# InfiniteNightmare/HNSW-Slim

Measured on AMD Instinct MI355X. Metric: QPS @ recall@10>=0.95 (SIFT-1M d=128, k=10), higher is better.
Workload: dtype f32

## Files before the change

hnsw-slim_amd/__init__.py:

```python
import ctypes
import os
import subprocess

import numpy as np

_HERE = os.path.dirname(os.path.abspath(__file__))
LIB_PATH = os.environ.get("HS_LIB", os.path.join(_HERE, "libhnsw_slim_amd.so"))

HS_KIND_HNSW, HS_KIND_SLIM, HS_KIND_SLIMQ = 0, 1, 2
HS_METRIC_L2, HS_METRIC_IP = 0, 1
HS_MODE_SLIM_IDS, HS_MODE_PQ = 0, 1
HS_ROWS_F32, HS_ROWS_F16, HS_ROWS_U8 = 0, 1, 2
HS_OK, HS_ERR_IO, HS_ERR_CORRUPT, HS_ERR_NOMEM, HS_ERR_INVALID, HS_ERR_UNSUPPORTED, HS_ERR_DEVICE, HS_ERR_CAPACITY = range(8)

EXPORTS = [
    "hs_last_error", "hs_device_count", "hs_index_load", "hs_index_load_mem", "hs_index_free", "hs_set_ef", "hs_index_info",
    "hs_set_capacity", "hs_set_exact_order", "hs_search_batch", "hs_search_batch_dev", "hs_search_check", "hs_search_batch_raw", "hs_search_batch_filtered", "hs_labels",
    "hs_build_hnsw", "hs_build_hnsw_labeled", "hs_convert_slim", "hs_rabitq_rotate", "hs_rabitq_quantize_data", "hs_rabitq_prepare_query",
    "hs_rabitq_estimate", "hs_convert_slimq", "hs_rabitq_default_tconst", "hs_slimq_set_dataset", "hs_slimq_set_tconst", "hs_slimq_get_tconst",
    "hs_slimq_search_batch", "hs_slimq_search_batch_dev", "hs_slimq_trace", "hs_slimq_prepare_debug", "hs_brute_force", "hs_brute_force_dev",
    "hs_search_batch_async", "hs_host_alloc", "hs_host_free", "hs_comm_init", "hs_comm_free", "hs_comm_size", "hs_search_batch_sharded",
    "hs_comm_results_dev", "hs_convert_slim_gpu", "hs_index_patch", "hs_index_from_host_arrays", "hs_build_rabitq_hnsw",
    "hs_convert_slimq_graph", "hs_host_device_pointer", "hs_index_set_row_format", "hs_index_row_format", "hs_rows_representable",
]
# ... 22 lines not shown


def lib():
    global _lib
    if _lib is not None:
        return _lib
    if not os.path.exists(LIB_PATH):
        raise HsError(HS_ERR_DEVICE, f"{LIB_PATH} is missing: build it with `make -C hnsw-slim_amd` "
                      "(__graft_entry__.build()); there is no CPU fallback")
    L = ctypes.CDLL(LIB_PATH)
    vp, sz, ci, u32 = ctypes.c_void_p, ctypes.c_size_t, ctypes.c_int, ctypes.c_uint32
    L.hs_last_error.restype = ctypes.c_char_p
    L.hs_device_count.restype = ci
    L.hs_index_load.argtypes = [ctypes.c_char_p, ci, ci, sz, sz, ci, ctypes.POINTER(vp)]
    L.hs_index_load_mem.argtypes = [ctypes.c_char_p, sz, ci, ci, sz, sz, ci, ctypes.POINTER(vp)]
    L.hs_index_patch.argtypes = [vp, ctypes.c_char_p, sz, ci]
    L.hs_index_from_host_arrays.argtypes = [ci, ci, sz, sz, vp, vp, vp, vp, vp, vp, u32, ctypes.c_int32, ctypes.c_int32, ci, ctypes.POINTER(vp)]
    L.hs_index_free.argtypes = [vp]
    L.hs_index_free.restype = None
    L.hs_set_ef.argtypes = [vp, sz]
    L.hs_index_info.argtypes = [vp, ctypes.POINTER(HsInfo)]
    L.hs_index_set_row_format.argtypes = [vp, ci]
    L.hs_index_row_format.argtypes = [vp]
    L.hs_rows_representable.argtypes = [vp, sz, sz, ci, ctypes.POINTER(ctypes.c_uint64)]
    L.hs_last_kernel.argtypes = [vp]
    L.hs_last_kernel.restype = ctypes.c_char_p
    L.hs_set_capacity.argtypes = [vp, u32, u32]
    L.hs_set_exact_order.argtypes = [vp, ci]
    L.hs_search_batch.argtypes = [vp, vp, sz, sz, ci, vp, vp, vp, vp, vp]
    L.hs_search_batch_dev.argtypes = [vp, vp, sz, sz, ci, vp, vp, vp, vp, vp, vp]
    L.hs_search_check.argtypes = [vp, vp]
    L.hs_debug_heap_ops.argtypes = [vp, sz, ci, u32, vp, vp, vp]
    L.hs_debug_flat_plan.argtypes = [sz, sz, sz, vp]
    L.hs_search_batch_async.argtypes = [vp, vp, sz, sz, ci, vp, vp, vp, vp, vp, vp]
    L.hs_host_alloc.restype = vp
    L.hs_host_alloc.argtypes = [sz]
    L.hs_host_free.restype = None
    L.hs_host_free.argtypes = [vp]
    L.hs_comm_init.argtypes = [ci, vp, ctypes.POINTER(vp)]
    L.hs_comm_free.restype = None
    L.hs_comm_free.argtypes = [vp]
    L.hs_comm_size.argtypes = [vp]
    L.hs_search_batch_sharded.argtypes = [vp, vp, vp, sz, sz, ci, vp, vp, vp, vp]
    L.hs_search_batch_sharded_async.argtypes = [vp, vp, vp, sz, sz, ci, vp, vp, vp, vp, ci]
    L.hs_comm_check.argtypes = [vp, vp, ci]
    L.hs_comm_slots.argtypes = [vp]
    L.hs_comm_results_dev.argtypes = [vp, ci, vp, vp, vp, vp]
    L.hs_search_batch_raw.argtypes = [vp, vp, sz, sz, ci, vp, vp, vp, vp]
    L.hs_search_batch_filtered.argtypes = [vp, vp, sz, sz, vp, vp, vp, vp, vp]
    L.hs_labels.argtypes = [vp, vp]
    L.hs_build_hnsw.argtypes = [vp, sz, sz, ci, sz, sz, ctypes.c_char_p, sz, ci, ctypes.c_char_p]
    L.hs_convert_slim.argtypes = [ctypes.c_char_p, ci, sz, ci, ctypes.c_float, ctypes.c_float, sz, sz, sz, sz, ci, ctypes.c_char_p]
    L.hs_convert_slimq_graph.argtypes = L.hs_convert_slim.argtypes
    L.hs_host_device_pointer.restype = ctypes.c_void_p
    L.hs_host_device_pointer.argtypes = [vp]
    L.hs_build_rabitq_hnsw.argtypes = [vp, sz, sz, ci, sz, sz, sz, ci, ctypes.c_char_p]
    L.hs_convert_slim_gpu.argtypes = [ctypes.c_char_p, ci, sz, ci, ctypes.c_float, ctypes.c_float, sz, sz, sz, sz, ci, ci, ctypes.c_char_p,
                                      ctypes.POINTER(ci), ctypes.POINTER(ctypes.c_double)]
    L.hs_convert_slimq.argtypes = [ctypes.c_char_p, ci, sz, vp, sz, vp, ctypes.c_uint64, ci, ctypes.c_char_p]
    L.hs_rabitq_default_tconst.restype = ctypes.c_double
    L.hs_rabitq_default_tconst.argtypes = [sz, ctypes.c_uint64]
    L.hs_slimq_set_dataset.argtypes = [vp, vp, sz, sz]
    L.hs_slimq_set_tconst.argtypes = [vp, ctypes.c_double]
    L.hs_slimq_get_tconst.restype = ctypes.c_double
    L.hs_slimq_get_tconst.argtypes = [vp]
    L.hs_slimq_search_batch.argtypes = [vp, vp, sz, sz, vp, vp, vp, vp]
# ... 49 lines not shown
    _check(lib().hs_convert_slim_gpu(hnsw_path.encode(), metric, dim, threshold_level, top_degree_percent0, top_degree_percent,
                                     top_degree_M0, low_degree_m0, top_degree_M, low_degree_m, device, threads, out_path.encode(),
                                     ctypes.byref(used), ctypes.byref(ms)))
    return bool(used.value), ms.value


def rows_representable(rows, fmt):
    r = np.ascontiguousarray(rows, np.float32)
    r = r.reshape(r.shape[0], -1) if r.ndim != 2 else r
    bad = ctypes.c_uint64(0)
    _check(lib().hs_rows_representable(r.ctypes.data, r.shape[0], r.shape[1], int(fmt), ctypes.byref(bad)))
    return None if bad.value == r.shape[0] else int(bad.value)


def debug_flat_plan(n, ef, nq):
    out = np.zeros(5, np.uint32)
    _check(lib().hs_debug_flat_plan(n, ef, nq, out.ctypes.data))
    return dict(nb=int(out[0]), mul=int(out[1]), sh=int(out[2]), bits=int(out[3]), ok=bool(out[4]))


def debug_heap_ops(ops, wave_pop=True, lds_slots=1024):
    n = len(ops)
    arr = np.zeros((max(n, 1), 3), np.uint32)
    for i, (kind, d, idv) in enumerate(ops):
        arr[i] = (kind, np.float32(d).view(np.uint32), idv)
    heap = np.zeros((n + 2, 2), np.uint32)
    pops = np.zeros((n + 2, 2), np.uint32)
    cnt = np.zeros(2, np.uint32)
    _check(lib().hs_debug_heap_ops(arr.ctypes.data, n, 1 if wave_pop else 0, lds_slots, heap.ctypes.data, pops.ctypes.data, cnt.ctypes.data))
    f = lambda a, m: [(float(a[i, 0:1].view(np.float32)[0]), int(a[i, 1])) for i in range(m)]
    return f(heap, int(cnt[0])), f(pops, int(cnt[1]))


def brute_force(base, queries, k, metric=HS_METRIC_L2, labels=None, device=0):
    b = np.ascontiguousarray(base, np.float32)
    q = np.ascontiguousarray(queries, np.float32)
    lab = None if labels is None else np.ascontiguousarray(labels, np.uint64)
    ol = np.empty((q.shape[0], k), np.uint64)
    od = np.empty((q.shape[0], k), np.float32)
    oc = np.empty(q.shape[0], np.uint32)
    _check(lib().hs_brute_force(b.ctypes.data, b.shape[0], b.shape[1], metric, None if lab is None else lab.ctypes.data, q.ctypes.data,
                                q.shape[0], k, device, ol.ctypes.data, od.ctypes.data, oc.ctypes.data))
    return ol, od, oc


def brute_force_dev(d_base, d_queries, k, d_labels_out, d_dists_out, metric=HS_METRIC_L2, d_counts=None, stream=0):
    _check(lib().hs_brute_force_dev(d_base.data_ptr(), None, d_base.shape[0], d_base.shape[1], metric, d_queries.data_ptr(),
                                    d_queries.shape[0], k, d_labels_out.data_ptr(), d_dists_out.data_ptr(),
                                    d_counts.data_ptr() if d_counts is not None else None, stream))


def convert_slimq(slim_path, metric, dim, centroids, out_path, cluster_ids=None, flip_seed=1, threads=8):
    c = np.ascontiguousarray(centroids, np.float32).reshape(-1, dim)
    cid = None if cluster_ids is None else np.ascontiguousarray(cluster_ids, np.uint32)
    _check(lib().hs_convert_slimq(slim_path.encode(), metric, dim, c.ctypes.data, c.shape[0], None if cid is None else cid.ctypes.data,
                                  flip_seed, threads, out_path.encode()))


def rabitq_default_tconst(padded_dim, seed=1):
    return lib().hs_rabitq_default_tconst(padded_dim, seed)


def rabitq_rotate(dim, flips, x):
    x = np.ascontiguousarray(x, np.float32)
    padded = (dim + 63) // 64 * 64
    flips = np.ascontiguousarray(flips, np.uint8)
# ... 312 lines not shown
```

hnsw-slim_amd/csrc/capi.cpp:

```cpp
#include <hip/hip_runtime.h>

#include <dlfcn.h>

#include <algorithm>
#include <cmath>
#include <cstdio>
#include <cstdlib>
#include <cstring>
#include <limits>
#include <map>
#include <memory>
#include <mutex>
#include <string>
#include <vector>

#include "../../include/hnsw_slim_amd.h"
#include "engine.hpp"
#include "narrow_rows.hpp"
#define HS_HAVE_GPU_CONVERT 1
#include "convert_engine.hpp"
#include "host_graph.hpp"
#include "rabitq_est.hpp"
#include "rabitq_host.hpp"
#include "slimq_engine.hpp"
// ... 671 lines not shown
}
int hs_index_row_format(const hs_index *ix) { return ix ? ix->row_fmt : ROWS_F32; }
hs_status hs_rows_representable(const float *rows, size_t n, size_t dim, int format, uint64_t *first_bad) {
  if (!first_bad || (n && dim && !rows)) return fail(HS_ERR_INVALID, "null argument");
  if (format != ROWS_F32 && format != ROWS_F16 && format != ROWS_U8) return fail(HS_ERR_INVALID, "bad row format");
  *first_bad = dim ? first_unfit(rows, n * dim, format) / dim : n;
  return HS_OK;
}

static constexpr size_t kMaxLaunchQueries = 32768;
static constexpr size_t kOrderMinQueries = 6144;

static hs_status search_dev_group(hs_index *ix, const float *d_q, size_t nq, size_t k, int mode, uint32_t *l32,
                                  uint64_t *l64, float *dd, uint32_t *cnt, uint32_t *stats, Pair *raw, uint32_t *rawsz,
                                  hipStream_t stream, bool first_group, size_t nq_total) {
  if (!ix) return fail(HS_ERR_INVALID, "null index");
  if (k == 0) return fail(HS_ERR_INVALID, "k must be > 0");
  if (mode != HS_MODE_SLIM_IDS && mode != HS_MODE_PQ) return fail(HS_ERR_INVALID, "bad mode");
  if (ix->info.kind == HS_KIND_SLIMQ) return fail(HS_ERR_INVALID, "SlimQ index: use hs_slimq_search_batch");
  if (mode == HS_MODE_SLIM_IDS && ix->info.kind != HS_KIND_SLIM)
    return fail(HS_ERR_INVALID, "HS_MODE_SLIM_IDS needs a Slim index (searchKnn(q,k,tableint*) exists on HierarchicalNSWSlim only)");
  if (nq > 0x7FFFFFFFu) return fail(HS_ERR_INVALID, "nq too large");
  if (nq == 0) return HS_OK;
  Shape sh;
  hs_status ps = plan_shape(ix, k, sh);
  if (ps != HS_OK) return ps;
  HIP_TRY(hipSetDevice(ix->device));
  hs_index::StreamWs *w = ix->stream_ws(stream);
  HIP_TRY(w->status.ensure(nq));
  HIP_TRY(w->spill.ensure(nq * (size_t)spill_stride_for(sh.ef)));
  if (w->counters.n < 48) {
    HIP_TRY(w->counters.ensure(48));
    HIP_TRY(hipMemsetAsync(w->counters.p, 0, 48 * sizeof(uint32_t), stream));
  } else {
    HIP_TRY(hipMemsetAsync(w->counters.p + 12, 0, sizeof(uint32_t), stream));
  }
  if (first_group) w->last_nq += nq_total;
  SearchArgs a{};
  a.queries = d_q; a.nq = (uint32_t)nq; a.k = (uint32_t)k; a.ef = sh.ef;
  a.cand_cap = sh.cand_cap; a.hash_slots = sh.hash_slots; a.mode = mode;
  a.mark_ep = (ix->info.kind == HS_KIND_SLIM && mode == HS_MODE_PQ) ? 1 : 0;
  a.out_labels32 = l32; a.out_labels64 = l64; a.out_dists = dd; a.out_counts = cnt; a.stats = stats;
  a.raw_top = raw; a.raw_size = rawsz; a.raw_stride = sh.ef;
  a.status = w->status.p;
  a.spill = w->spill.p; a.spill_slots = kSpillSlots; a.spill_stride = spill_stride_for(sh.ef); a.cand2_cap = kCand2Cap;
  a.log_cap = log_cap_for(sh.ef); a.hop_cap = hop_cap_for(sh.ef);
  static const bool flat_off = getenv("HS_FLAT") && atoi(getenv("HS_FLAT")) == 0;
  a.flat = flat_off ? 0u : 1u;
  if (sh.q_bits && !ix->user_hash_slots) {
    const size_t waves_per_cu = std::max<size_t>((nq + 255) / 256, 1);
    const size_t budget = std::min<size_t>(kLdsPerCU / waves_per_cu, 64 * 1024);
    uint32_t bbits = 0;
    while ((1u << bbits) < sh.q_hash_slots / 4) bbits++;
    for (int step = 0; step < 2; step++) {
      const uint32_t bigger = sh.q_hash_slots * 2;
      const size_t lds_fast = fast_lds_bytes((uint32_t)ix->info.dim, sh.ef, sh.cand_cap_fast, bigger);
      const size_t lds_lean = lean_lds_bytes((uint32_t)ix->info.dim, sh.ef, sh.l_cand_cap, bigger);
      if (std::max(lds_fast, lds_lean) > budget || bbits + 1 > sh.q_bits) break;
      sh.q_hash_slots = bigger;
      bbits++;
    }
  }
  const uint32_t fast_hash = sh.q_bits ? sh.q_hash_slots : sh.hash_slots;
  const bool fast = !ix->exact_order && !raw && fast_supported(ix->dev, sh.ef, (uint32_t)k) &&
                    fast_lds_bytes((uint32_t)ix->info.dim, sh.ef, sh.cand_cap_fast, fast_hash) <= kLdsPerCU;
  auto fast_scratch = [&](bool on) {
    a.cand_cap = on ? sh.cand_cap_fast : sh.cand_cap;
    a.hash_slots = on ? fast_hash : sh.hash_slots;
    a.vis_bits = on ? sh.q_bits : 0;
  };
  static const char *kernel_env = getenv("HS_KERNEL");
  static const bool lean_forced = getenv("HS_LEAN_MIN_EF") != nullptr;
  static const uint32_t lean_min_ef = lean_forced ? (uint32_t)atoi(getenv("HS_LEAN_MIN_EF")) : kLeanMinEf;
  static const bool lean_asked = lean_forced || (kernel_env && !strcmp(kernel_env, "lean"));
  const bool lean = lean_asked && fast && sh.ef >= lean_min_ef && lean_supported(ix->dev, sh.ef, (uint32_t)k) &&
                    lean_lds_bytes((uint32_t)ix->info.dim, sh.ef, sh.l_cand_cap, sh.q_bits ? sh.q_hash_slots : sh.l_hash_slots) <= kLdsPerCU;
  static const bool flatk_off = kernel_env && (!strcmp(kernel_env, "lean") || !strcmp(kernel_env, "fast"));
  const FlatPlan fp = plan_flat(ix, sh.ef, nq);
  const bool flatk = !flatk_off && !lean_forced && fast && fp.ok && flatk_supported(ix->dev, sh.ef, (uint32_t)k);
  const bool narrow = flatk && ix->row_fmt != ROWS_F32;
  auto flat_go = [&]() { return narrow ? launch_flatk_narrow(ix->dev, a, ix->narrow.p, ix->row_fmt, stream) : launch_flatk(ix->dev, a, stream); };
  ix->last_kernel = narrow ? (ix->row_fmt == ROWS_U8 ? "hs::flat_kernel_u8" : "hs::flat_kernel_f16") : flatk ? "hs::flat_kernel" : lean ? "hs::lean_kernel" : fast ? "hs::fast_kernel" : "hs::strict_kernel";
  a.queue = w->counters.p + 12;
  a.counters = w->counters.p; a.pass_id = 0;
  static const int order_env = getenv("HS_ORDER") ? atoi(getenv("HS_ORDER")) : -1;
  const bool ordered = fast && (order_env < 0 ? nq >= kOrderMinQueries : order_env != 0);
  if (flatk) {
    a.hash_slots = fp.nb * 4; a.vis_bits = fp.vis_bits; a.fl_nb = fp.nb; a.fl_mul = fp.mul; a.fl_sh = fp.sh;
    a.select_mask = 1u << ST_TODO; a.grid = (uint32_t)nq;
    if (ordered) {
      HIP_TRY(w->entry.ensure(nq * 4));
      HIP_TRY(w->order.ensure(nq));
      a.entry = reinterpret_cast<uint4 *>(w->entry.p); a.order = w->order.p;
      a.phase = 1;
      HIP_TRY(flat_go());
      HIP_TRY(launch_order(a.entry, w->order.p, (uint32_t)nq, stream));
      a.phase = 2;
      HIP_TRY(flat_go());
      a.phase = 0;
    } else {
      HIP_TRY(flat_go());
    }
    a.cand_cap = sh.cand_cap; a.hash_slots = sh.hash_slots; a.vis_bits = 0;
  } else if (lean) {
    a.cand_cap = sh.l_cand_cap; a.hash_slots = sh.q_bits ? sh.q_hash_slots : sh.l_hash_slots; a.hash_fill_shift = 3; a.vis_bits = sh.q_bits;
    a.select_mask = 1u << ST_TODO; a.grid = (uint32_t)nq;
    if (ordered) {
      HIP_TRY(w->entry.ensure(nq * 4));
      HIP_TRY(w->order.ensure(nq));
      a.entry = reinterpret_cast<uint4 *>(w->entry.p); a.order = w->order.p;
      a.phase = 1;
      HIP_TRY(launch_lean(ix->dev, a, stream));
      HIP_TRY(launch_order(a.entry, w->order.p, (uint32_t)nq, stream));
      a.phase = 2;
      HIP_TRY(launch_lean(ix->dev, a, stream));
      a.phase = 0;
// ... 68 lines not shown
    return HS_OK;
  }
  if (c[8] + c[9] > 0)
    return fail(HS_ERR_CAPACITY, std::to_string(c[8] + c[9]) + " queries exhausted even a whole CU's on-chip scratch");
  return HS_OK;
}

hs_status hs_debug_flat_plan(size_t n, size_t ef, size_t nq, uint32_t *out5) {
  if (!out5) return fail(HS_ERR_INVALID, "null argument");
  hs_index tmp;
  tmp.info.n = n; tmp.info.dim = 128;
  const FlatPlan f = plan_flat(&tmp, (uint32_t)ef, nq);
  out5[0] = f.nb; out5[1] = f.mul; out5[2] = f.sh; out5[3] = f.vis_bits; out5[4] = f.ok ? 1u : 0u;
  return HS_OK;
}

hs_status hs_debug_heap_ops(const uint32_t *ops, size_t n_ops, int wave_pop, uint32_t lds_slots, uint32_t *out_heap, uint32_t *out_pops,
                            uint32_t *out_n) {
  if (!ops || !out_heap || !out_pops || !out_n) return fail(HS_ERR_INVALID, "null argument");
  if (lds_slots < 2 || lds_slots > 8192 || (lds_slots & 1)) return fail(HS_ERR_INVALID, "lds_slots: even, 2..8192");
  DevBuf<uint32_t> d_ops, d_n;
  DevBuf<uint2> d_spill, d_heap, d_pops;
  HIP_TRY(d_ops.alloc(std::max<size_t>(3 * n_ops, 1)));
  HIP_TRY(d_n.alloc(2));
  HIP_TRY(d_spill.alloc(n_ops + 2));
  HIP_TRY(d_heap.alloc(n_ops + 2));
  HIP_TRY(d_pops.alloc(n_ops + 2));
  HIP_TRY(hipMemcpy(d_ops.p, ops, 3 * n_ops * sizeof(uint32_t), hipMemcpyHostToDevice));
  HIP_TRY(flat_heap_ops(d_ops.p, (uint32_t)n_ops, d_spill.p, d_heap.p, d_pops.p, d_n.p, wave_pop, lds_slots, nullptr));
  HIP_TRY(hipDeviceSynchronize());
  HIP_TRY(hipMemcpy(out_n, d_n.p, 8, hipMemcpyDeviceToHost));
  HIP_TRY(hipMemcpy(out_heap, d_heap.p, (size_t)out_n[0] * 8, hipMemcpyDeviceToHost));
  HIP_TRY(hipMemcpy(out_pops, d_pops.p, (size_t)out_n[1] * 8, hipMemcpyDeviceToHost));
  return HS_OK;
}

hs_status hs_search_batch_dev(hs_index *ix, const float *d_queries, size_t nq, size_t k, int mode,
                              uint32_t *d_out_labels32, uint64_t *d_out_labels64, float *d_out_dists,
                              uint32_t *d_out_counts, uint32_t *d_stats, void *stream) {
  if (mode == HS_MODE_SLIM_IDS && !d_out_labels32) return fail(HS_ERR_INVALID, "out_labels32 required");
  if (mode == HS_MODE_PQ && (!d_out_labels64 || !d_out_dists || !d_out_counts)) return fail(HS_ERR_INVALID, "out_labels64/out_dists/out_counts required");
  return search_dev(ix, d_queries, nq, k, mode, d_out_labels32, d_out_labels64, d_out_dists, d_out_counts, d_stats,
                    nullptr, nullptr, (hipStream_t)stream);
}

static void *mapped_device_pointer(const void *host) {
  if (!host) return nullptr;
  hipPointerAttribute_t at{};
  if (hipPointerGetAttributes(&at, host) != hipSuccess) { (void)hipGetLastError(); return nullptr; }
  if (at.type != hipMemoryTypeHost || !at.devicePointer) return nullptr;
  return at.devicePointer;
}
static constexpr size_t kZeroCopyQueryBytes = 2u << 20;
static hs_status search_async(hs_index *ix, const float *queries, size_t nq, size_t k, int mode, uint32_t *l32, uint64_t *l64,
                              float *dd, uint32_t *cnt, uint32_t *stats, hipStream_t st) {
  if (!ix || !queries) return fail(HS_ERR_INVALID, "null argument");
  if (k == 0) return fail(HS_ERR_INVALID, "k must be > 0");
  if (nq == 0) return HS_OK;
  HIP_TRY(hipSetDevice(ix->device));
  const size_t dim = ix->info.dim;
  hs_index::StreamWs *w = ix->stream_ws(st);
  static const bool zero_copy_off = getenv("HS_ZERO_COPY") && !strcmp(getenv("HS_ZERO_COPY"), "0");
  static const bool zero_copy_in_only = getenv("HS_ZERO_COPY") && !strcmp(getenv("HS_ZERO_COPY"), "in");
  const bool ids = mode == HS_MODE_SLIM_IDS;
  const float *dq = nullptr;
  if (!zero_copy_off && nq * dim * sizeof(float) <= kZeroCopyQueryBytes) dq = static_cast<const float *>(mapped_device_pointer(queries));
// ... 804 lines not shown
```

hnsw-slim_amd/csrc/engine.hpp:

```cpp
#pragma once
#include <hip/hip_runtime.h>

#include <cstdint>

#include "heap_emul.hpp"

namespace hs {

struct DevIndex {
  const float *vec;
  const uint32_t *row_ptr0;
  const uint32_t *cols;
  const uint32_t *up_base;
  const uint32_t *up_ptr;
  const uint32_t *tile0;
  const uint2 *uptile;
  const uint64_t *labels;
  const uint8_t *deleted;
  uint32_t n, dim, tile_stride, up_stride, ep_base;
  int32_t maxlevel, threshold_level;
  uint32_t enterpoint;
  int32_t has_deleted, kind, metric;
};

enum : uint32_t { ST_TODO = 0, ST_DONE = 1, ST_OVERFLOW = 2, ST_HAZARD = 3 };

struct SearchArgs {
  const float *queries;
  uint32_t nq, k, ef;
  uint32_t cand_cap;
  uint32_t hash_slots;
  uint32_t *spill;
  uint32_t spill_slots, spill_stride, cand2_cap, log_cap;
  int32_t mode;
  int32_t mark_ep;
  uint32_t select_mask;
  uint32_t grid;
  uint32_t *out_labels32;
  uint64_t *out_labels64;
  float *out_dists;
  uint32_t *out_counts;
  uint32_t *stats;
  Pair *raw_top;
  uint32_t *raw_size;
  uint32_t raw_stride;
  uint32_t *status;
  uint32_t *counters;
  uint32_t pass_id;
  uint32_t *queue;
  uint32_t hash_fill_shift;
  uint32_t flat;
  uint32_t hop_cap;
  uint32_t vis_bits;
  uint32_t phase;
  uint4 *entry;
  const uint32_t *order;
  void *fb_cand;
  uint32_t *fb_spill;
  uint32_t fl_nb, fl_mul, fl_sh;
};

size_t strict_lds_bytes(uint32_t dim, uint32_t ef, uint32_t cand_cap, uint32_t hash_slots);
size_t fast_lds_bytes(uint32_t dim, uint32_t ef, uint32_t cand_cap, uint32_t hash_slots);
bool fast_supported(const DevIndex &ix, uint32_t ef, uint32_t k);

hipError_t launch_strict(const DevIndex &ix, const SearchArgs &a, hipStream_t stream);
hipError_t launch_order(const uint4 *entry, uint32_t *order, uint32_t nq, hipStream_t stream);
bool lean_supported(const DevIndex &ix, uint32_t ef, uint32_t k);
size_t lean_lds_bytes(uint32_t dim, uint32_t ef, uint32_t cand_cap, uint32_t hash_slots);
hipError_t launch_lean(const DevIndex &ix, const SearchArgs &a, hipStream_t stream);
bool flatk_supported(const DevIndex &ix, uint32_t ef, uint32_t k);
size_t flatk_lds_bytes(uint32_t dim, uint32_t ef, uint32_t nb);
uint32_t flatk_waves_per_cu(uint32_t dim, uint32_t ef);
hipError_t launch_flatk(const DevIndex &ix, const SearchArgs &a, hipStream_t stream);
hipError_t flat_heap_ops(const uint32_t *d_ops, uint32_t n_ops, uint2 *d_spill, uint2 *d_heap, uint2 *d_pops, uint32_t *d_n, int wave_pop,
                         uint32_t lds_slots, hipStream_t stream);
hipError_t launch_fast(const DevIndex &ix, const SearchArgs &a, hipStream_t stream);
hipError_t launch_flatk_narrow(const DevIndex &ix, const SearchArgs &a, const void *rows, int fmt, hipStream_t stream);
hipError_t launch_narrow_convert(const float *d_vec, void *d_out, int fmt, uint32_t row0, uint32_t nrows, uint32_t dim, uint32_t *d_first_bad,
                                 hipStream_t stream);

}
```

hnsw-slim_amd/csrc/flat_search.hip:

```cpp
#include <hip/hip_runtime.h>

#include <algorithm>
#include <cfloat>
#include <climits>

#include "dist_recipe.hpp"
#include "engine.hpp"
#include "heap_emul.hpp"
#include "search_common.hpp"
#include "wave_util.hpp"

namespace hs {

typedef __attribute__((address_space(3))) unsigned char lds_u8;
typedef __attribute__((address_space(3))) uint32_t lds_u32;
typedef __attribute__((address_space(3))) unsigned short lds_u16;
typedef uint32_t hs_u4 __attribute__((ext_vector_type(4)));
typedef __attribute__((address_space(3))) hs_u4 lds_u128;
typedef __attribute__((address_space(3))) float lds_f32;
typedef __attribute__((address_space(3))) hs_f2 lds_f2;
typedef unsigned short hs_us2 __attribute__((ext_vector_type(2)));

static constexpr uint32_t kFlatOvfCap = 64;
static constexpr uint32_t kFlatBucketTags = 7;
// ... 363 lines not shown
    }
    hq++;
  }
  bool stop = rc != 0 || cand_size == 0;
  if (!stop) {
    const uint2 root = fh_get<false>(cand, 1);
    const uint32_t rkey_bits = uni(root.x);
    if (dkey<METRIC>(__uint_as_float(rkey_bits)) > lb) {
      stop = true;
    } else {
      next_id = uni(root.y);
      if (cand_size < heap_lds_slots) fh_pop_wave(cand, cand_size, lane);
      else if (lane == 0) fh_pop<true>(cand, cand_size);
      cand_size--;
      hp++;
      wave_sync();
    }
  }
  for (uint32_t sl = lane; sl <= cand_size && sl < heap_lds_slots; sl += 64) {
    const hs_u2 e = *reinterpret_cast<lds_u64 *>(vis + sl * 8);
    heap_store[sl] = make_uint2(e.x, e.y);
  }
  wave_sync();
  __threadfence_block();
  for (uint32_t i = lane; i * 2u < heap_lds_slots; i += 64) *reinterpret_cast<lds_u128 *>(vis + i * 16) = park[i];
  wave_sync();
  FlatSyncOut o;
  o.cand_size = cand_size; o.hp = hp; o.hq = hq; o.h_idx = h_idx; o.rc = rc; o.stop = stop ? 1u : 0u; o.next_id = next_id;
  return o;
}

template <int S>
__device__ __forceinline__ int rank_key(const int (&tk)[S], uint32_t r) {
  const uint32_t l = r / S, sl = r % S;
  int v = __builtin_amdgcn_readlane(tk[0], l);
#pragma unroll
  for (int s = 1; s < S; s++) {
    const int t = __builtin_amdgcn_readlane(tk[s], l);
    v = sl == (uint32_t)s ? t : v;
  }
  return v;
}
template <int S>
__device__ __forceinline__ uint32_t rank_id(const uint32_t (&ti)[S], uint32_t r) {
  const uint32_t l = r / S, sl = r % S;
  uint32_t v = __builtin_amdgcn_readlane(ti[0], l);
#pragma unroll
  for (int s = 1; s < S; s++) {
    const uint32_t t = __builtin_amdgcn_readlane(ti[s], l);
    v = sl == (uint32_t)s ? t : v;
  }
  return v;
}

template <int METRIC, int S, int D16, typename ROW>
__device__ int search_one_flat(const DevIndex &ix, const SearchArgs &a, const uint32_t qi, lds_u8 *smem, const ROW *rows) {
  const int lane = threadIdx.x;
  constexpr int OWN = METRIC == METRIC_L2 ? 7 : 0;
  const int s8 = lane & 7, grp = lane >> 3;
  const uint32_t dim = D16 > 0 ? (uint32_t)D16 * 16u : ix.dim;
  const FlatLds L = flat_layout(dim, a.ef, a.fl_nb);
  lds_u8 *qv = smem + L.off_q;
  lds_u8 *vis = smem + L.off_vis;
  lds_u32 *ovf = reinterpret_cast<lds_u32 *>(smem + L.off_ovf);
  lds_u32 *nid = reinterpret_cast<lds_u32 *>(smem + L.off_nid);
  const uint32_t k = a.k, ef = a.ef;
  uint32_t *scratch = a.spill + (size_t)qi * a.spill_stride;
  uint2 *tlog = reinterpret_cast<uint2 *>(scratch + a.spill_slots + 2 * a.cand2_cap);
  uint32_t *hoplog = scratch + a.spill_slots + 2 * a.cand2_cap + 2 * a.log_cap;
  const uint32_t hop_cap = a.hop_cap / 4;
  uint32_t n_dist = 1, n_hops = 0, n_nbr = 0;
#ifdef HS_FLAT_DIAG
  const unsigned long long diag_t0 = __builtin_amdgcn_s_memrealtime();
  uint32_t diag_syncs = 0, diag_replayed = 0, diag_sync_ticks = 0, diag_pre = 0;
  uint32_t diag_ph[6] = {0, 0, 0, 0, 0, 0};
  unsigned long long diag_tp = __builtin_amdgcn_s_memtime();
#define HS_DIAG_LAP(i) { const unsigned long long t_ = __builtin_amdgcn_s_memtime(); diag_ph[i] += (uint32_t)(t_ - diag_tp); diag_tp = t_; }
#else
#define HS_DIAG_LAP(i)
#endif

  for (uint32_t i = lane; i < dim; i += 64) reinterpret_cast<lds_f32 *>(qv)[i] = a.queries[(size_t)qi * dim + i];
  for (uint32_t i = lane; i < a.fl_nb; i += 64) *reinterpret_cast<lds_u128 *>(vis + i * 16) = hs_u4{~0u, ~0u, ~0u, 0x0000FFFFu};
  uint32_t ovf_n = 0;
  const uint32_t vmask = a.vis_bits >= 32 ? 0xFFFFFFFFu : (1u << a.vis_bits) - 1u;
// ... 262 lines not shown
      const int my_key = (s8 == OWN && act) ? dkey<METRIC>(d) : kFKeyInf;
#ifdef HS_FLAT_DIAG
      asm volatile("s_nop 0" : : "v"(my_key) : "memory");
      HS_DIAG_LAP(3);
#endif
      int b_lane = -1;
      if (base + 8 >= cnt && ghost_key != lb) {
        const Near u = nearest();
        int mk = min(my_key, __builtin_amdgcn_update_dpp(kFKeyInf, my_key, 0x118, 0xf, 0xf, false));
        const int b_key = min(min(__builtin_amdgcn_readlane(mk, OWN + 8), __builtin_amdgcn_readlane(mk, OWN + 24)),
                              min(__builtin_amdgcn_readlane(mk, OWN + 40), __builtin_amdgcn_readlane(mk, OWN + 56)));
        const bool b_ok = b_key < lb;
        if (b_ok && (!u.any || b_key < u.key)) {
          const unsigned long long bm = hs_ballot(my_key == b_key);
          if (__popcll(bm) == 1) {
            b_lane = __ffsll((long long)bm) - 1;
            have_pre = true;
            pre_key = b_key;
            pre_id = __builtin_amdgcn_readlane(rid, b_lane);
          }
        } else if (u.any && u.same == 1 && (!b_ok || u.key < b_key)) {
          const uint32_t below = __popcll(hs_ballot(my_key < u.key));
          if ((uint32_t)(u.p * S + u.slot) + below < ef) {
            have_pre = true;
            pre_key = u.key;
            pre_id = u.id;
#pragma unroll
            for (int s = 0; s < S; s++) ti[s] = ti[s] == pre_id ? (pre_id | kFDone) : ti[s];
          }
        }
        pre_tile = kNone;
        if (have_pre && (uint32_t)lane < stride) pre_tile = ix.tile0[(size_t)pre_id * stride + lane];
      }
      unsigned long long todo = hs_ballot(my_key < lb);
      unsigned long long am = 0;
      while (todo) {
        const int jl = __ffsll((long long)todo) - 1;
        todo &= todo - 1;
        const int kj = __builtin_amdgcn_readlane(my_key, jl);
        if (kj < lb) {
          const uint32_t idj = __builtin_amdgcn_readlane(rid, jl) | (jl == b_lane ? kFDone : 0u);
          am |= 1ull << jl;
          uint32_t pos = 0;
#pragma unroll
          for (int s = 0; s < S; s++) pos += __popcll(hs_ballot(tk[s] <= kj));
          const int ek = lb;
          uint32_t ei = 0;
          if (exact_fit) ei = rank_id<S>(ti, ef - 1);
          const int upk = __builtin_amdgcn_update_dpp(0, tk[S - 1], 0x138, 0xf, 0xf, false);
          const uint32_t upi = (uint32_t)__builtin_amdgcn_update_dpp(0, (int)ti[S - 1], 0x138, 0xf, 0xf, false);
#pragma unroll
          for (int s = S - 1; s >= 1; s--) {
            const bool gt = (uint32_t)(laneS + s) > pos;
            tk[s] = gt ? tk[s - 1] : tk[s];
            ti[s] = gt ? ti[s - 1] : ti[s];
          }
          {
            const bool gt = (uint32_t)laneS > pos;
            tk[0] = gt ? upk : tk[0];
            ti[0] = gt ? upi : ti[0];
          }
          {
            const uint32_t pl = pos / S, ps = pos % S;
#pragma unroll
            for (int s = 0; s < S; s++)
              if (ps == (uint32_t)s) {
                tk[s] = (int)write_lane((uint32_t)tk[s], (uint32_t)kj, pl);
                ti[s] = write_lane(ti[s], idj, pl);
              }
          }
          lb = rank_key<S>(tk, ef - 1);
          if (exact_fit && ek != kFKeyInf && lb == ek) {
            btie = true;
            if ((int)ei >= 0) ghost_key = ek;
          }
        }
      }
      if (am) {
        const uint32_t at = n_log + __popcll(am & ((1ull << lane) - 1ull));
        if (((am >> lane) & 1ull) && at < a.log_cap) tlog[at] = make_uint2(__float_as_uint(d), rid);
        const uint32_t na = __popcll(am);
        n_log += na;
        n_acc_hop += na;
      }
      HS_DIAG_LAP(4);
    }
    if (!exact_fit && n_acc_hop != 0 && lb != kFKeyInf) {
      unsigned long long eq = 0, un = 0;
#pragma unroll
      for (int s = 0; s < S; s++) {
        const unsigned long long e = hs_ballot(tk[s] == lb) & ~inr[s];
        eq |= e;
        un |= e & hs_ballot((int)ti[s] >= 0);
      }
      if (eq) btie = true;
      if (un) ghost_key = lb;
      if (__builtin_expect(rank_key<S>(tk, 64 * S - 1) == lb, 0)) { rc = 3; break; }
    }
    hl = write_lane(hl, uni(n_acc_hop), uni(hop0 & 63u));
    hop0++;
    if (__builtin_expect((hop0 & 63u) == 0, 0)) {
      if (hop0 > hop_cap) { rc = 3; break; }
      hoplog[hop0 - 64 + lane] = hl;
    }
    if (__builtin_expect(n_log > a.log_cap, 0)) { rc = 3; break; }
    HS_DIAG_LAP(5);
  }
  if (__builtin_expect(rc == 1 || rc == 2, 0)) {
    flag_query(a, qi, ST_OVERFLOW, rc - 1, lane);
    return rc;
// ... 145 lines not shown
__global__ void __launch_bounds__(64) flat_heap_ops_kernel(const uint32_t *ops, uint32_t n_ops, uint2 *spill, uint2 *out_heap, uint2 *out_pops,
                                                            uint32_t *out_n, int wave_pop, uint32_t lds_slots) {
  extern __shared__ __align__(16) unsigned char smem_raw[];
  const int lane = threadIdx.x;
  FlatHeap h;
  h.lds = (lds_u8 *)smem_raw;
  h.L = lds_slots;
  h.glob = spill;
  uint32_t size = 0, pops = 0;
  for (uint32_t i = 0; i < n_ops; i++) {
    const uint32_t kind = uni(ops[3 * i]), key = uni(ops[3 * i + 1]), id = uni(ops[3 * i + 2]);
    if (kind == 0) {
      size++;
      if (size < h.L) fh_push<false>(h, size, __uint_as_float(key), id, lane);
      else fh_push<true>(h, size, __uint_as_float(key), id, lane);
    } else if (size > 0) {
      const uint2 root = fh_get<true>(h, 1);
      if (lane == 0) out_pops[pops] = root;
      pops++;
      if (wave_pop && size < h.L) fh_pop_wave(h, size, lane);
      else if (lane == 0) { if (size < h.L) fh_pop<false>(h, size); else fh_pop<true>(h, size); }
      size--;
    }
    wave_sync();
  }
  for (uint32_t s = lane; s < size; s += 64) out_heap[s] = fh_get<true>(h, s + 1);
  if (lane == 0) { out_n[0] = size; out_n[1] = pops; }
}
hipError_t flat_heap_ops(const uint32_t *d_ops, uint32_t n_ops, uint2 *d_spill, uint2 *d_heap, uint2 *d_pops, uint32_t *d_n, int wave_pop,
                         uint32_t lds_slots, hipStream_t stream) {
  hipLaunchKernelGGL(flat_heap_ops_kernel, dim3(1), dim3(64), (size_t)lds_slots * 8, stream, d_ops, n_ops, d_spill, d_heap, d_pops, d_n, wave_pop, lds_slots);
  return hipGetLastError();
}
#endif

hipError_t launch_flatk_l2(const DevIndex &ix, const SearchArgs &a, hipStream_t stream);
hipError_t launch_flatk_ip(const DevIndex &ix, const SearchArgs &a, hipStream_t stream);
#if !defined(HS_TU_METRIC) || HS_TU_METRIC == 0
bool flatk_supported(const DevIndex &ix, uint32_t ef, uint32_t k) {
  return ix.tile0 != nullptr && (ix.maxlevel == 0 || ix.uptile != nullptr) && ix.threshold_level == 0 && !ix.has_deleted && ix.n > 0 &&
         ix.n < kFDone && (ix.dim & 15u) == 0 && ef >= k && ef <= 512 && k <= 64;
}
uint32_t flatk_waves_per_cu(uint32_t dim, uint32_t ef) {
  const int s = ef <= 64 ? 1 : ef <= 128 ? 2 : ef <= 192 ? 3 : ef <= 256 ? 4 : ef <= 384 ? 6 : 8;
  const int d16 = dim == 128 ? 8 : dim == 96 ? 6 : dim == 960 ? 60 : dim > 256 ? -1 : 0;
  return 4u * (uint32_t)flat_waves(s, d16);
}
size_t flatk_lds_bytes(uint32_t dim, uint32_t ef, uint32_t nb) { return flat_layout(dim, ef, nb).total; }
hipError_t launch_flatk_l2(const DevIndex &ix, const SearchArgs &a, hipStream_t stream) { return flat_launch_s<METRIC_L2>(ix, a, nullptr, stream); }
hipError_t launch_flatk(const DevIndex &ix, const SearchArgs &a, hipStream_t stream) {
  return ix.metric == METRIC_L2 ? launch_flatk_l2(ix, a, stream) : launch_flatk_ip(ix, a, stream);
}
#endif
#if !defined(HS_TU_METRIC) || HS_TU_METRIC == 1
hipError_t launch_flatk_ip(const DevIndex &ix, const SearchArgs &a, hipStream_t stream) { return flat_launch_s<METRIC_IP>(ix, a, nullptr, stream); }
#endif
#elif HS_TU_ROWS == 1
#if !defined(HS_TU_METRIC) || HS_TU_METRIC == 0
hipError_t launch_flatk_u8_l2(const DevIndex &ix, const SearchArgs &a, const void *rows, hipStream_t stream) { return flat_launch_s<METRIC_L2>(ix, a, rows, stream); }
#endif
#if !defined(HS_TU_METRIC) || HS_TU_METRIC == 1
hipError_t launch_flatk_u8_ip(const DevIndex &ix, const SearchArgs &a, const void *rows, hipStream_t stream) { return flat_launch_s<METRIC_IP>(ix, a, rows, stream); }
#endif
#else
#if !defined(HS_TU_METRIC) || HS_TU_METRIC == 0
hipError_t launch_flatk_f16_l2(const DevIndex &ix, const SearchArgs &a, const void *rows, hipStream_t stream) { return flat_launch_s<METRIC_L2>(ix, a, rows, stream); }
// ... 8 lines not shown
```

include/hnsw_slim_amd.h:

```cpp
#ifndef HNSW_SLIM_AMD_H
#define HNSW_SLIM_AMD_H

#include <stddef.h>
#include <stdint.h>

#ifdef __cplusplus
extern "C" {
#endif

typedef struct hs_index hs_index;

typedef enum {
  HS_OK = 0,
  HS_ERR_IO = 1,
  HS_ERR_CORRUPT = 2,
  HS_ERR_NOMEM = 3,
  HS_ERR_INVALID = 4,
  HS_ERR_UNSUPPORTED = 5,
  HS_ERR_DEVICE = 6,
  HS_ERR_CAPACITY = 7
} hs_status;

typedef enum { HS_KIND_HNSW = 0, HS_KIND_SLIM = 1, HS_KIND_SLIMQ = 2 } hs_kind;
typedef enum { HS_METRIC_L2 = 0, HS_METRIC_IP = 1 } hs_metric;
// ... 26 lines not shown
                                    const uint8_t *deleted, const int32_t *levels, const uint64_t *list_ptr,
                                    const uint32_t *list_ids, uint32_t enterpoint, int32_t maxlevel, int32_t threshold_level,
                                    int device, hs_index **out);
hs_status hs_index_patch(hs_index *ix, const void *bytes, size_t len, int to_add);
typedef enum { HS_ROWS_F32 = 0, HS_ROWS_F16 = 1, HS_ROWS_U8 = 2 } hs_row_format;
hs_status hs_index_set_row_format(hs_index *ix, int format);
int hs_index_row_format(const hs_index *ix);
hs_status hs_rows_representable(const float *rows, size_t n, size_t dim, int format, uint64_t *first_bad);
void hs_index_free(hs_index *ix);
hs_status hs_set_ef(hs_index *ix, size_t ef);
hs_status hs_index_info(const hs_index *ix, hs_info *out);
const char *hs_last_kernel(const hs_index *ix);

hs_status hs_set_exact_order(hs_index *ix, int on);

hs_status hs_set_capacity(hs_index *ix, uint32_t cand_cap, uint32_t hash_slots);

hs_status hs_search_batch(hs_index *ix, const float *queries, size_t nq, size_t k, int mode,
                          uint32_t *out_labels32, uint64_t *out_labels64, float *out_dists,
                          uint32_t *out_counts, uint32_t *stats);

hs_status hs_search_batch_filtered(hs_index *ix, const float *queries, size_t nq, size_t k,
                                   const uint8_t *allowed, uint64_t *out_labels64, float *out_dists,
                                   uint32_t *out_counts, uint32_t *stats);
hs_status hs_labels(const hs_index *ix, uint64_t *out_labels);

hs_status hs_search_batch_dev(hs_index *ix, const float *d_queries, size_t nq, size_t k, int mode,
                              uint32_t *d_out_labels32, uint64_t *d_out_labels64, float *d_out_dists,
                              uint32_t *d_out_counts, uint32_t *d_stats, void *stream);
hs_status hs_search_check(hs_index *ix, void *stream);
hs_status hs_debug_flat_plan(size_t n, size_t ef, size_t nq, uint32_t *out5);
hs_status hs_debug_heap_ops(const uint32_t *ops, size_t n_ops, int wave_pop, uint32_t lds_slots, uint32_t *out_heap, uint32_t *out_pops,
                            uint32_t *out_n);

hs_status hs_search_batch_async(hs_index *ix, const float *queries, size_t nq, size_t k, int mode,
                                uint32_t *out_labels32, uint64_t *out_labels64, float *out_dists,
                                uint32_t *out_counts, uint32_t *stats, void *stream);
void *hs_host_alloc(size_t bytes);
void hs_host_free(void *p);
void *hs_host_device_pointer(const void *host);

typedef struct hs_comm hs_comm;
hs_status hs_comm_init(int n_gpus, const int *devices, hs_comm **out);
void hs_comm_free(hs_comm *c);
int hs_comm_size(const hs_comm *c);
hs_status hs_search_batch_sharded(hs_comm *c, hs_index *const *ixs, const float *queries, size_t nq, size_t k, int mode,
                                  uint32_t *out_labels32, uint64_t *out_labels64, float *out_dists, uint32_t *out_counts);
int hs_comm_slots(const hs_comm *c);
hs_status hs_search_batch_sharded_async(hs_comm *c, hs_index *const *ixs, const float *queries, size_t nq, size_t k, int mode,
                                        uint32_t *out_labels32, uint64_t *out_labels64, float *out_dists, uint32_t *out_counts, int slot);
hs_status hs_comm_check(hs_comm *c, hs_index *const *ixs, int slot);
hs_status hs_comm_results_dev(hs_comm *c, int rank, const uint32_t **d_labels32, const uint64_t **d_labels64,
                              const float **d_dists, const uint32_t **d_counts);

hs_status hs_search_batch_raw(hs_index *ix, const float *queries, size_t nq, size_t k, int mode,
                              float *raw_dists, uint32_t *raw_ids, uint32_t *raw_sizes, uint32_t *stats);

hs_status hs_slimq_set_dataset(hs_index *ix, const float *base, size_t n, size_t dim);
hs_status hs_slimq_set_tconst(hs_index *ix, double t_const);
double hs_slimq_get_tconst(const hs_index *ix);
hs_status hs_slimq_search_batch(hs_index *ix, const float *queries, size_t nq, size_t k, uint64_t *out_labels,
                                float *out_dists, uint32_t *out_counts, uint32_t *stats);
hs_status hs_slimq_search_batch_dev(hs_index *ix, const float *d_queries, size_t nq, size_t k, uint64_t *d_out_labels,
                                    float *d_out_dists, uint32_t *d_out_counts, uint32_t *d_stats, void *stream);

hs_status hs_slimq_prepare_debug(hs_index *ix, const float *queries, size_t nq, float *out);
// ... 47 lines not shown
```

Baseline: 13.90 million.

## Batch candidate acceptance in flat kernel with two-phase rank-then-insert pass

Replaces the per-candidate serial insert loop in the flat search kernel with a two-phase pass. The first phase computes each accepted candidate's final position from ballots over both the existing list and the batch itself. The second phase inserts the candidates with a single combined shift-and-write per candidate, and the lower bound is recomputed only once per pass instead of after every insertion. It also drops the unused per-call queue counter memset and field, and adds a debug entry point plus kernel so the acceptance logic can be tested. The new scheme changes how tie tracking is handled, so it risks small behavioral differences when the list is exactly full.

```diff
diff --git a/hnsw-slim_amd/__init__.py b/hnsw-slim_amd/__init__.py
--- a/hnsw-slim_amd/__init__.py
+++ b/hnsw-slim_amd/__init__.py
@@ -78,6 +78,8 @@
     L.hs_search_check.argtypes = [vp, vp]
     L.hs_debug_heap_ops.argtypes = [vp, sz, ci, u32, vp, vp, vp]
     L.hs_debug_flat_plan.argtypes = [sz, sz, sz, vp]
+    if hasattr(L, "hs_debug_flat_accept"):
+        L.hs_debug_flat_accept.argtypes = [vp, vp, vp, sz, u32, vp, vp, vp, vp]
     L.hs_search_batch_async.argtypes = [vp, vp, sz, sz, ci, vp, vp, vp, vp, vp, vp]
     L.hs_host_alloc.restype = vp
     L.hs_host_alloc.argtypes = [sz]
@@ -193,6 +195,27 @@
     return f(heap, int(cnt[0])), f(pops, int(cnt[1]))
 
 
+FLAT_KEY_INF = 0x7F800000
+FLAT_DONE = 0x80000000
+
+
+def debug_flat_accept(keys, ids, flag, ef):
+    k = np.ascontiguousarray(keys, np.int32).reshape(-1, 8)
+    i = np.ascontiguousarray(ids, np.uint32).reshape(-1, 8)
+    f = np.ascontiguousarray(flag, np.int32).reshape(-1)
+    n = k.shape[0]
+    assert i.shape[0] == n and f.shape[0] == n
+    cap = 64 * (1 if ef <= 64 else 2 if ef <= 128 else 3 if ef <= 192 else 4 if ef <= 256 else 6 if ef <= 384 else 8)
+    ok = np.zeros((n, cap), np.int32)
+    oi = np.zeros((n, cap), np.uint32)
+    am = np.zeros(n, np.uint32)
+    lb = np.zeros((n, 3), np.int32)
+    _check(lib().hs_debug_flat_accept(k.ctypes.data, i.ctypes.data, f.ctypes.data, n, ef, ok.ctypes.data, oi.ctypes.data,
+                                      am.ctypes.data, lb.ctypes.data))
+    acc = ((am[:, None] >> np.arange(8, dtype=np.uint32)[None, :]) & 1).astype(bool)
+    return ok, oi, acc, lb
+
+
 def brute_force(base, queries, k, metric=HS_METRIC_L2, labels=None, device=0):
     b = np.ascontiguousarray(base, np.float32)
     q = np.ascontiguousarray(queries, np.float32)
diff --git a/hnsw-slim_amd/csrc/capi.cpp b/hnsw-slim_amd/csrc/capi.cpp
--- a/hnsw-slim_amd/csrc/capi.cpp
+++ b/hnsw-slim_amd/csrc/capi.cpp
@@ -727,8 +727,6 @@
   if (w->counters.n < 48) {
     HIP_TRY(w->counters.ensure(48));
     HIP_TRY(hipMemsetAsync(w->counters.p, 0, 48 * sizeof(uint32_t), stream));
-  } else {
-    HIP_TRY(hipMemsetAsync(w->counters.p + 12, 0, sizeof(uint32_t), stream));
   }
   if (first_group) w->last_nq += nq_total;
   SearchArgs a{};
@@ -776,7 +774,6 @@
   const bool narrow = flatk && ix->row_fmt != ROWS_F32;
   auto flat_go = [&]() { return narrow ? launch_flatk_narrow(ix->dev, a, ix->narrow.p, ix->row_fmt, stream) : launch_flatk(ix->dev, a, stream); };
   ix->last_kernel = narrow ? (ix->row_fmt == ROWS_U8 ? "hs::flat_kernel_u8" : "hs::flat_kernel_f16") : flatk ? "hs::flat_kernel" : lean ? "hs::lean_kernel" : fast ? "hs::fast_kernel" : "hs::strict_kernel";
-  a.queue = w->counters.p + 12;
   a.counters = w->counters.p; a.pass_id = 0;
   static const int order_env = getenv("HS_ORDER") ? atoi(getenv("HS_ORDER")) : -1;
   const bool ordered = fast && (order_env < 0 ? nq >= kOrderMinQueries : order_env != 0);
@@ -911,6 +908,34 @@
   HIP_TRY(hipMemcpy(out_n, d_n.p, 8, hipMemcpyDeviceToHost));
   HIP_TRY(hipMemcpy(out_heap, d_heap.p, (size_t)out_n[0] * 8, hipMemcpyDeviceToHost));
   HIP_TRY(hipMemcpy(out_pops, d_pops.p, (size_t)out_n[1] * 8, hipMemcpyDeviceToHost));
+  return HS_OK;
+}
+
+hs_status hs_debug_flat_accept(const int32_t *keys, const uint32_t *ids, const int32_t *flag, size_t n_pass, uint32_t ef, int32_t *out_keys,
+                               uint32_t *out_ids, uint32_t *out_am, int32_t *out_lb) {
+  if (!keys || !ids || !flag || !out_keys || !out_ids || !out_am || !out_lb) return fail(HS_ERR_INVALID, "null argument");
+  if (ef < 1 || ef > 512 || n_pass < 1 || n_pass > (1u << 20)) return fail(HS_ERR_INVALID, "ef: 1..512, n_pass: 1..2^20");
+  for (size_t p = 0; p < n_pass; p++)
+    if (flag[p] < -1 || flag[p] > 7) return fail(HS_ERR_INVALID, "flag: -1..7");
+  const size_t cap = 64 * (size_t)(ef <= 64 ? 1 : ef <= 128 ? 2 : ef <= 192 ? 3 : ef <= 256 ? 4 : ef <= 384 ? 6 : 8);
+  DevBuf<int> d_keys, d_flag, d_ok, d_lb;
+  DevBuf<uint32_t> d_ids, d_oi, d_am;
+  HIP_TRY(d_keys.alloc(8 * n_pass));
+  HIP_TRY(d_ids.alloc(8 * n_pass));
+  HIP_TRY(d_flag.alloc(n_pass));
+  HIP_TRY(d_ok.alloc(cap * n_pass));
+  HIP_TRY(d_oi.alloc(cap * n_pass));
+  HIP_TRY(d_am.alloc(n_pass));
+  HIP_TRY(d_lb.alloc(3 * n_pass));
+  HIP_TRY(hipMemcpy(d_keys.p, keys, 8 * n_pass * sizeof(int), hipMemcpyHostToDevice));
+  HIP_TRY(hipMemcpy(d_ids.p, ids, 8 * n_pass * sizeof(uint32_t), hipMemcpyHostToDevice));
+  HIP_TRY(hipMemcpy(d_flag.p, flag, n_pass * sizeof(int), hipMemcpyHostToDevice));
+  HIP_TRY(flat_accept_ops(d_keys.p, d_ids.p, d_flag.p, (uint32_t)n_pass, ef, d_ok.p, d_oi.p, d_am.p, d_lb.p, nullptr));
+  HIP_TRY(hipDeviceSynchronize());
+  HIP_TRY(hipMemcpy(out_keys, d_ok.p, cap * n_pass * sizeof(int), hipMemcpyDeviceToHost));
+  HIP_TRY(hipMemcpy(out_ids, d_oi.p, cap * n_pass * sizeof(uint32_t), hipMemcpyDeviceToHost));
+  HIP_TRY(hipMemcpy(out_am, d_am.p, n_pass * sizeof(uint32_t), hipMemcpyDeviceToHost));
+  HIP_TRY(hipMemcpy(out_lb, d_lb.p, 3 * n_pass * sizeof(int), hipMemcpyDeviceToHost));
   return HS_OK;
 }
 
diff --git a/hnsw-slim_amd/csrc/engine.hpp b/hnsw-slim_amd/csrc/engine.hpp
--- a/hnsw-slim_amd/csrc/engine.hpp
+++ b/hnsw-slim_amd/csrc/engine.hpp
@@ -47,7 +47,6 @@
   uint32_t *status;
   uint32_t *counters;
   uint32_t pass_id;
-  uint32_t *queue;
   uint32_t hash_fill_shift;
   uint32_t flat;
   uint32_t hop_cap;
@@ -75,6 +74,8 @@
 hipError_t launch_flatk(const DevIndex &ix, const SearchArgs &a, hipStream_t stream);
 hipError_t flat_heap_ops(const uint32_t *d_ops, uint32_t n_ops, uint2 *d_spill, uint2 *d_heap, uint2 *d_pops, uint32_t *d_n, int wave_pop,
                          uint32_t lds_slots, hipStream_t stream);
+hipError_t flat_accept_ops(const int *d_keys, const uint32_t *d_ids, const int *d_flag, uint32_t n_pass, uint32_t ef, int *d_out_keys,
+                           uint32_t *d_out_ids, uint32_t *d_out_am, int *d_out_lb, hipStream_t stream);
 hipError_t launch_fast(const DevIndex &ix, const SearchArgs &a, hipStream_t stream);
 hipError_t launch_flatk_narrow(const DevIndex &ix, const SearchArgs &a, const void *rows, int fmt, hipStream_t stream);
 hipError_t launch_narrow_convert(const float *d_vec, void *d_out, int fmt, uint32_t row0, uint32_t nrows, uint32_t dim, uint32_t *d_first_bad,
diff --git a/hnsw-slim_amd/csrc/flat_search.hip b/hnsw-slim_amd/csrc/flat_search.hip
--- a/hnsw-slim_amd/csrc/flat_search.hip
+++ b/hnsw-slim_amd/csrc/flat_search.hip
@@ -419,7 +419,9 @@
 
 template <int S>
 __device__ __forceinline__ int rank_key(const int (&tk)[S], uint32_t r) {
-  const uint32_t l = r / S, sl = r % S;
+  const uint32_t l = r / S;
+  uint32_t sl = r % S;
+  if constexpr (S > 1) asm volatile("" : "+s"(sl));
   int v = __builtin_amdgcn_readlane(tk[0], l);
 #pragma unroll
   for (int s = 1; s < S; s++) {
@@ -438,6 +440,65 @@
     v = sl == (uint32_t)s ? t : v;
   }
   return v;
+}
+
+template <int S>
+__device__ __forceinline__ void flat_insert_at(int (&tk)[S], uint32_t (&ti)[S], const int laneS, const uint32_t pos, const int kj, const uint32_t idj) {
+  const int upk = __builtin_amdgcn_update_dpp(0, tk[S - 1], 0x138, 0xf, 0xf, false);
+  const uint32_t upi = (uint32_t)__builtin_amdgcn_update_dpp(0, (int)ti[S - 1], 0x138, 0xf, 0xf, false);
+#pragma unroll
+  for (int s = S - 1; s >= 0; s--) {
+    const bool ge = (uint32_t)(laneS + s) >= pos, gt = (uint32_t)(laneS + s) > pos;
+    const int pk = s > 0 ? tk[s > 0 ? s - 1 : 0] : upk;
+    const uint32_t pi = s > 0 ? ti[s > 0 ? s - 1 : 0] : upi;
+    tk[s] = ge ? (gt ? pk : kj) : tk[s];
+    ti[s] = ge ? (gt ? pi : idj) : ti[s];
+  }
+}
+
+template <int S>
+__device__ __forceinline__ unsigned long long flat_accept_pass(int (&tk)[S], uint32_t (&ti)[S], const int my_key, const uint32_t rid, const int b_lane,
+                                                               const uint32_t ef, const int laneS, int &lb, bool &btie, int &ghost_key) {
+  const unsigned long long cm = hs_ballot(my_key < lb);
+  if (cm == 0) return 0;
+  unsigned long long am = 0;
+  uint32_t kv = (uint32_t)my_key;
+  unsigned long long todo = cm;
+  while (todo) {
+    const int jl = __ffsll((long long)todo) - 1;
+    todo &= todo - 1;
+    const int kj = __builtin_amdgcn_readlane(kv, jl);
+    uint32_t pos = __popcll(hs_ballot((int)kv <= kj) & cm & ((1ull << jl) - 1ull));
+#pragma unroll
+    for (int s = 0; s < S; s++) pos += __popcll(hs_ballot(tk[s] <= kj));
+    if (pos < ef) {
+      am |= 1ull << jl;
+      kv = write_lane(kv, pos, (uint32_t)jl ^ 1u);
+    }
+  }
+  if (am == 0) return 0;
+  const bool exact_fit = ef == 64u * S;
+  todo = am;
+  while (todo) {
+    const int jl = __ffsll((long long)todo) - 1;
+    todo &= todo - 1;
+    const uint32_t pos = __builtin_amdgcn_readlane(kv, jl ^ 1);
+    const int kj = __builtin_amdgcn_readlane(kv, jl);
+    const uint32_t idj = __builtin_amdgcn_readlane(rid, jl) | (jl == b_lane ? kFDone : 0u);
+    int ek = kFKeyInf;
+    uint32_t ei = 0;
+    if (exact_fit) {
+      ek = __builtin_amdgcn_readlane(tk[S - 1], 63);
+      ei = __builtin_amdgcn_readlane(ti[S - 1], 63);
+    }
+    flat_insert_at<S>(tk, ti, laneS, pos, kj, idj);
+    if (exact_fit && ek != kFKeyInf && __builtin_amdgcn_readlane(tk[S - 1], 63) == ek) {
+      btie = true;
+      if ((int)ei >= 0) ghost_key = ek;
+    }
+  }
+  lb = rank_key<S>(tk, ef - 1);
+  return am;
 }
 
 template <int METRIC, int S, int D16, typename ROW>
@@ -766,50 +827,7 @@
         pre_tile = kNone;
         if (have_pre && (uint32_t)lane < stride) pre_tile = ix.tile0[(size_t)pre_id * stride + lane];
       }
-      unsigned long long todo = hs_ballot(my_key < lb);
-      unsigned long long am = 0;
-      while (todo) {
-        const int jl = __ffsll((long long)todo) - 1;
-        todo &= todo - 1;
-        const int kj = __builtin_amdgcn_readlane(my_key, jl);
-        if (kj < lb) {
-          const uint32_t idj = __builtin_amdgcn_readlane(rid, jl) | (jl == b_lane ? kFDone : 0u);
-          am |= 1ull << jl;
-          uint32_t pos = 0;
-#pragma unroll
-          for (int s = 0; s < S; s++) pos += __popcll(hs_ballot(tk[s] <= kj));
-          const int ek = lb;
-          uint32_t ei = 0;
-          if (exact_fit) ei = rank_id<S>(ti, ef - 1);
-          const int upk = __builtin_amdgcn_update_dpp(0, tk[S - 1], 0x138, 0xf, 0xf, false);
-          const uint32_t upi = (uint32_t)__builtin_amdgcn_update_dpp(0, (int)ti[S - 1], 0x138, 0xf, 0xf, false);
-#pragma unroll
-          for (int s = S - 1; s >= 1; s--) {
-            const bool gt = (uint32_t)(laneS + s) > pos;
-            tk[s] = gt ? tk[s - 1] : tk[s];
-            ti[s] = gt ? ti[s - 1] : ti[s];
-          }
-          {
-            const bool gt = (uint32_t)laneS > pos;
-            tk[0] = gt ? upk : tk[0];
-            ti[0] = gt ? upi : ti[0];
-          }
-          {
-            const uint32_t pl = pos / S, ps = pos % S;
-#pragma unroll
-            for (int s = 0; s < S; s++)
-              if (ps == (uint32_t)s) {
-                tk[s] = (int)write_lane((uint32_t)tk[s], (uint32_t)kj, pl);
-                ti[s] = write_lane(ti[s], idj, pl);
-              }
-          }
-          lb = rank_key<S>(tk, ef - 1);
-          if (exact_fit && ek != kFKeyInf && lb == ek) {
-            btie = true;
-            if ((int)ei >= 0) ghost_key = ek;
-          }
-        }
-      }
+      const unsigned long long am = flat_accept_pass<S>(tk, ti, my_key, rid, b_lane, ef, laneS, lb, btie, ghost_key);
       if (am) {
         const uint32_t at = n_log + __popcll(am & ((1ull << lane) - 1ull));
         if (((am >> lane) & 1ull) && at < a.log_cap) tlog[at] = make_uint2(__float_as_uint(d), rid);
@@ -1021,6 +1039,50 @@
   hipLaunchKernelGGL(flat_heap_ops_kernel, dim3(1), dim3(64), (size_t)lds_slots * 8, stream, d_ops, n_ops, d_spill, d_heap, d_pops, d_n, wave_pop, lds_slots);
   return hipGetLastError();
 }
+static int flat_slots(uint32_t ef) { return ef <= 64 ? 1 : ef <= 128 ? 2 : ef <= 192 ? 3 : ef <= 256 ? 4 : ef <= 384 ? 6 : 8; }
+template <int S>
+__global__ void __launch_bounds__(64) flat_accept_ops_kernel(const int *keys, const uint32_t *ids, const int *flag, uint32_t n_pass, uint32_t ef,
+                                                              int *out_keys, uint32_t *out_ids, uint32_t *out_am, int *out_lb) {
+  const int lane = threadIdx.x, laneS = lane * S;
+  int tk[S];
+  uint32_t ti[S];
+#pragma unroll
+  for (int s = 0; s < S; s++) {
+    tk[s] = kFKeyInf;
+    ti[s] = kFDone;
+  }
+  int lb = rank_key<S>(tk, ef - 1), ghost_key = INT_MIN;
+  bool btie = false;
+  for (uint32_t p = 0; p < n_pass; p++) {
+    const bool own = (lane & 7) == 7;
+    const int my_key = own ? keys[8 * p + (lane >> 3)] : kFKeyInf;
+    const uint32_t rid = ids[8 * p + (lane >> 3)];
+    const int f = (int)uni((uint32_t)flag[p]);
+    const unsigned long long am = flat_accept_pass<S>(tk, ti, my_key, rid, f < 0 ? -1 : 8 * f + 7, ef, laneS, lb, btie, ghost_key);
+    uint32_t bits = 0;
+    for (int g = 0; g < 8; g++) bits |= (uint32_t)((am >> (8 * g + 7)) & 1ull) << g;
+#pragma unroll
+    for (int s = 0; s < S; s++) {
+      out_keys[(size_t)p * 64 * S + laneS + s] = tk[s];
+      out_ids[(size_t)p * 64 * S + laneS + s] = ti[s];
+    }
+    if (lane == 0) { out_am[p] = bits; out_lb[3 * p] = lb; out_lb[3 * p + 1] = ghost_key; out_lb[3 * p + 2] = btie ? 1 : 0; }
+  }
+}
+hipError_t flat_accept_ops(const int *d_keys, const uint32_t *d_ids, const int *d_flag, uint32_t n_pass, uint32_t ef, int *d_out_keys,
+                           uint32_t *d_out_ids, uint32_t *d_out_am, int *d_out_lb, hipStream_t stream) {
+#define HS_ACCEPT_OPS(S) hipLaunchKernelGGL(flat_accept_ops_kernel<S>, dim3(1), dim3(64), 0, stream, d_keys, d_ids, d_flag, n_pass, ef, d_out_keys, d_out_ids, d_out_am, d_out_lb)
+  switch (flat_slots(ef)) {
+    case 1: HS_ACCEPT_OPS(1); break;
+    case 2: HS_ACCEPT_OPS(2); break;
+    case 3: HS_ACCEPT_OPS(3); break;
+    case 4: HS_ACCEPT_OPS(4); break;
+    case 6: HS_ACCEPT_OPS(6); break;
+    default: HS_ACCEPT_OPS(8); break;
+  }
+#undef HS_ACCEPT_OPS
+  return hipGetLastError();
+}
 #endif
 
 hipError_t launch_flatk_l2(const DevIndex &ix, const SearchArgs &a, hipStream_t stream);
diff --git a/include/hnsw_slim_amd.h b/include/hnsw_slim_amd.h
--- a/include/hnsw_slim_amd.h
+++ b/include/hnsw_slim_amd.h
@@ -82,6 +82,8 @@
 hs_status hs_debug_flat_plan(size_t n, size_t ef, size_t nq, uint32_t *out5);
 hs_status hs_debug_heap_ops(const uint32_t *ops, size_t n_ops, int wave_pop, uint32_t lds_slots, uint32_t *out_heap, uint32_t *out_pops,
                             uint32_t *out_n);
+hs_status hs_debug_flat_accept(const int32_t *keys, const uint32_t *ids, const int32_t *flag, size_t n_pass, uint32_t ef, int32_t *out_keys,
+                               uint32_t *out_ids, uint32_t *out_am, int32_t *out_lb);
 
 hs_status hs_search_batch_async(hs_index *ix, const float *queries, size_t nq, size_t k, int mode,
                                 uint32_t *out_labels32, uint64_t *out_labels64, float *out_dists,
```

Result: slower. 13.44 million (-3.3%).
